# sherholz/mitsuba-path-guiding

Hardware: AMD Instinct MI355X
Metric: Mpaths/sec + equal-spp RMSE vs CPU ref, ajar-door scene at 1/2/4/8 GPUs (higher is better)
Workload: dtype f32; 1 GPU; C3 ajar_door 1280x720, guided SD-tree, 5 training iterations (1..16 spp) + 1024 spp render; scene=ajar_door, triangles=58864, width=1280, height=720, spp=1024, parallelism=tile-shard x1, no exchange (one rank)

## Files before the change

mitsuba-path-guiding_amd/csrc/pg_host.cpp:

```cpp
#include <hip/hip_runtime.h>
#include <rccl/rccl.h>

#include <algorithm>
#include <atomic>
#include <chrono>
#include <cmath>
#include <cstdio>
#include <cstdlib>
#include <cstring>
#include <limits>
#include <string>
#include <vector>

#include "../../include/pg_capi.h"
#include "pg_bvh.h"
#include "pg_envmap.h"
#include "pg_kernels.h"
#include "pg_layout.h"
#include "pg_rtrans.h"
#include "pg_sdtree.h"

namespace {

constexpr uint32_t kStackDepth = 48;
// ... 475 lines not shown
        (void)hipEventCreate(&e.b);
        pool.push_back(e);
    }
    return pool[l->evused[l->evcur]++];
}

bool raySortEnabled() {
    static const bool on = [] {
        const char *e = std::getenv("PG_RAY_SORT");
        return e && std::atoi(e) != 0;
    }();
    return on;
}
constexpr uint32_t kRaySortMinShard = 1024;

uint32_t tailPaths() {
    static const uint32_t n = [] {
        const char *e = std::getenv("PG_TAIL_PATHS");
        return e ? (uint32_t)std::strtoul(e, nullptr, 10) : (uint32_t)1 << 17;
    }();
    return n;
}

int vertexSlots(const Ctx *c, bool rec) { return rec ? std::max(0, std::min(c->cfg.record_max_vertices, 64)) : 0; }

void releasePaths(Ctx *c) {
    for (int li = 0; li < c->nlanes; ++li) {
        Lane &l = c->lanes[li];
        for (DevBuf *b : {&l.ray_o, &l.ray_d, &l.hit, &l.thr, &l.rad, &l.pinfo, &l.sh_d, &l.sh_c,
                          &l.vtx, &l.q0, &l.q1, &l.qs, &l.qp, &l.class_q, &l.aov, &l.qkey, &l.qsorted})
// ... 1302 lines not shown
    uint32_t nextLayer = 0, nextPix = 0, nextChunk = 0;
    uint32_t filmNext = 0;
    HIPC(c, hipEventRecord(c->pass_start, c->stream));
    HIPC(c, hipEventRecord(c->film_order, c->stream));
    c->rec_bound = c->rec_host_count;

    auto lqueue = [](const Lane &l, uint32_t *items, uint32_t *counts) {
        return Queue{items, counts, pg_queue_stride(l.P)};
    };
    auto classQueues = [&](const Lane &l, uint32_t *cb, Queue *cls) {
        for (int k = 0; k < PG_CLASS_ROWS; ++k)
            cls[k] = lqueue(l, k < PG_NUM_CLASSES ? l.class_q.as<uint32_t>() + (size_t)k * PG_QSHARDS * pg_queue_stride(l.P)
                                                 : nullptr,
                            cb + kClassCounts + k * PG_QSHARDS);
    };
    auto launchTrace = [&](Lane &l, const Queue *shq, const Queue *pq) -> pg_status {
        uint32_t *cb = l.counters.as<uint32_t>() + (size_t)kBounceWords * l.b;
        Queue cls[PG_CLASS_ROWS];
        classQueues(l, cb, cls);
        EventPair et{};
        if (evt) et = nextEvents(&l, shq ? KT_RAYS : KT_TRACE);
        if (evt) HIPC(c, hipEventRecord(et.a, l.stream));
        const Queue tq = lqueue(l, l.sorted ? l.qsorted.as<uint32_t>() : (l.b & 1) ? l.q1.as<uint32_t>() : l.q0.as<uint32_t>(),
                                cb);
        if (shq) pg_launch_rays(l.stream, g, sc, pathView(&l), tq, l.bound, cls, *shq, l.bound, *pq);
        else pg_launch_trace(l.stream, g, sc, pathView(&l), tq, l.bound, cls, l.b == 0);
        if (evt) HIPC(c, hipEventRecord(et.b, l.stream));
        HIPC(c, hipMemcpyAsync(l.h_counts + (size_t)kBounceWords * l.b + kClassCounts, cb + kClassCounts,
                               PG_CLASS_ROWS * PG_QSHARDS * 4, hipMemcpyDeviceToHost, l.stream));
        HIPC(c, hipEventRecord(l.ready, l.stream));
        return PG_OK;
    };
    auto collectStats = [&](Lane &l) -> pg_status {
        if (!l.stats_pending) return PG_OK;
        HIPC(c, hipEventSynchronize(l.done));
        for (uint32_t k = 0; k < l.stats_bounces; ++k)
            for (int sh = 0; sh < PG_QSHARDS; ++sh)
            {
                c->stats.shadow_rays += l.h_stats[(size_t)kBounceWords * k + kShadowCounts + sh];
                c->probes += l.h_stats[(size_t)kBounceWords * k + kProbeCounts + sh];
                c->stats.shadow_rays += l.h_stats[(size_t)kBounceWords * k + kDropCounts + sh];
// ... 45 lines not shown
        l.n = np * nl;
        nextPix += np;
        if (nextPix >= npix) {
            nextPix = 0;
            nextLayer += nl;
        }
        l.b = 0;
        l.sorted = false;
        l.bound = pg_camera_bound(pg_camera_banded(bands, l.np), l.np, l.nl);
        l.active = true;
        l.traced = false;
        l.chunk = nextChunk++;
        HIPC(c, hipStreamWaitEvent(l.stream, c->pass_start, 0));
        HIPC(c, hipMemsetAsync(l.counters.p, 0, (size_t)kBounceWords * (maxBounces + 1) * 4, l.stream));
        HIPC(c, hipMemsetAsync(l.tail_stats.p, 0, kTailStats * 8, l.stream));
        pg_launch_camera(l.stream, g, pathView(&l), c->d_band_pixels.as<uint32_t>(), l.pb, l.np, l.nl,
                         sample_offset + l.layer0, lqueue(l, l.q0.as<uint32_t>(), l.counters.as<uint32_t>()), bands);
        return launchTrace(l, nullptr, nullptr);
    };
    auto finishChunk = [&](Lane &l) -> pg_status {
        pg_status st;
        if ((st = collectStats(l))) return st;
        const PathDev pv = pathView(&l);
        HIPC(c, hipMemcpyAsync(l.h_stats, l.counters.p, (size_t)kBounceWords * l.b * 4, hipMemcpyDeviceToHost, l.stream));
        HIPC(c, hipMemcpyAsync(l.h_tail, l.tail_stats.p, kTailStats * 8, hipMemcpyDeviceToHost, l.stream));
        HIPC(c, hipStreamWaitEvent(l.stream, c->film_order, 0));
        pg_launch_film(l.stream, g, sc, pv, c->d_band_pixels.as<uint32_t>(), l.pb, l.np, l.nl, c->film.as<float4>(),
                       c->film_sq.as<float4>(), c->aov_albedo.as<float4>(), c->aov_normal.as<float4>());
        if (c->filtered)
            launchFilmFiltered(c, l.stream, g, sc, pv, c->d_band_pixels.as<uint32_t>(), l.pb, l.np, l.nl,
                               sample_offset + l.layer0);
        if (rec) {
// ... 43 lines not shown
            if (k < PG_NUM_CLASSES) clsMax[k] = m;
        }
        {
            uint64_t t = 0;
            for (int w = 0; w < PG_CLASS_ROWS * PG_QSHARDS; ++w) t += hc[w];
            l.used_cur.push_back(t);
        }
        ++l.b;
        const uint32_t tailMax = c->cfg.tail_paths < 0 ? 0u : c->cfg.tail_paths > 0 ? (uint32_t)c->cfg.tail_paths : tailPaths();
        const bool tail = nlive > 0 && nlive <= tailMax && l.b < maxBounces;
        if (tail) {
            const uint32_t *cbt = l.counters.as<uint32_t>() + (size_t)kBounceWords * (l.b - 1);
            const Queue tq = lqueue(l, l.sorted ? l.qsorted.as<uint32_t>()
                                                : ((l.b - 1) & 1) ? l.q1.as<uint32_t>() : l.q0.as<uint32_t>(),
                                    const_cast<uint32_t *>(cbt));
            pg_launch_tail(l.stream, g, sc, sd, pathView(&l), tq, l.bound, l.tail_stats.as<unsigned long long>());
            c->stats.tail_launches += 1;
        }
        if (nlive == 0 || tail || l.b >= maxBounces) {
            l.traced = true;
            for (bool progress = true; progress;) {
                progress = false;
                for (Lane &o : c->lanes)
                    if (o.active && o.traced && o.chunk == filmNext) {
                        ++filmNext;
                        pg_status st = finishChunk(o);
                        if (st) return st;
                        progress = true;
                    }
            }
            return PG_OK;
// ... 647 lines not shown
```

mitsuba-path-guiding_amd/csrc/pg_kernels.h:

```cpp
#pragma once
#include <hip/hip_runtime.h>
#include <stdint.h>

#include "pg_layout.h"

struct SceneDev {
    const float4 *nodes;
    const float4 *tris;
    const float4 *wnodes;
    const float4 *wtris;
    const float4 *tshade;
    const uint8_t *tclass;
    const GMat *mats;
    const GEmitter *ems;
    const float4 *emtri;
    const float *emcdf;
    const GEnv *env;
    uint32_t top_nodes;
    uint32_t num_em_boxes;
    float em_absmax;
    float em_box[PG_EMBOX_MAX][6];
    uint32_t num_blockers;
    float absmax;
    uint32_t *blk_counts;
// ... 65 lines not shown
struct Queue {
    uint32_t *items;
    uint32_t *counts;
    uint32_t stride;
    uint16_t *keys = nullptr;
    uint32_t *dropped = nullptr;
};
#define PG_RAY_SORT_BINS 4096
__host__ __device__ inline uint32_t pg_queue_stride(uint32_t capacity) {
    return 64u * ((capacity + 4095u) / 4096u + (uint32_t)(((uint64_t)capacity * 7u + (1u << 24) - 1u) >> 24) + 2u);
}
__host__ __device__ inline uint32_t pg_camera_shard_count(uint32_t n, uint32_t s) {
    int rem = (int)(n & 4095u) - 64 * (int)s;
    return 64u * (n >> 12) + (uint32_t)(rem < 0 ? 0 : rem > 64 ? 64 : rem);
}
constexpr uint32_t kBandMinPixels = 4096;
__host__ __device__ inline uint32_t pg_band_start(uint32_t r, uint32_t npix) {
    return (uint32_t)(((uint64_t)r * npix + 7u) / 8u);
}
__host__ __device__ inline uint32_t pg_banded_shard_count(uint32_t npix, uint32_t nlayers, uint32_t s) {
    const uint32_t r = s & 7u, j = s >> 3;
    const uint32_t m = (pg_band_start(r + 1, npix) - pg_band_start(r, npix)) * nlayers;
    const int rem = (int)(m & 511u) - 64 * (int)j;
    return 64u * (m >> 9) + (uint32_t)(rem < 0 ? 0 : rem > 64 ? 64 : rem);
}
__host__ __device__ inline bool pg_camera_banded(bool bands, uint32_t npix) { return bands && npix >= kBandMinPixels; }
__host__ __device__ inline uint32_t pg_camera_count(bool banded, uint32_t npix, uint32_t nlayers, uint32_t s) {
    return banded ? pg_banded_shard_count(npix, nlayers, s) : pg_camera_shard_count(npix * nlayers, s);
}
inline uint32_t pg_camera_bound(bool banded, uint32_t npix, uint32_t nlayers) {
    uint32_t b = 0;
    for (uint32_t s = 0; s < 64; ++s) {
        const uint32_t c = pg_camera_count(banded, npix, nlayers, s);
        b = c > b ? c : b;
    }
    return b;
}

void pg_launch_camera(hipStream_t s, const GParams &g, const PathDev &p, const uint32_t *local_pixels,
                      uint32_t pix_begin, uint32_t npix, uint32_t nlayers, uint32_t sample_base, Queue q, bool banded);
void pg_launch_trace(hipStream_t s, const GParams &g, const SceneDev &sc, const PathDev &p, Queue q, uint32_t max_shard,
                     const Queue *class_queues, bool first_bounce);
void pg_launch_shade_class(hipStream_t s, int cls, const GParams &g, const SceneDev &sc, const SDDev &sd,
                           const PathDev &p, Queue in, uint32_t max_shard, Queue out, Queue shadow, Queue probe);
void pg_launch_shade_all(hipStream_t s, const GParams &g, const SceneDev &sc, const SDDev &sd, const PathDev &p,
                         const Queue *class_queues, const uint32_t *max_shard, Queue out, Queue shq, Queue probe);
void pg_launch_rays(hipStream_t s, const GParams &g, const SceneDev &sc, const PathDev &p, Queue q, uint32_t max_shard,
                    const Queue *class_queues, Queue shq, uint32_t max_shadow_shard, Queue probe);
void pg_launch_shadow(hipStream_t s, const GParams &g, const SceneDev &sc, const PathDev &p, Queue q, uint32_t max_shard);
void pg_launch_probe(hipStream_t s, const SceneDev &sc, const PathDev &p, Queue probe, uint32_t max_shard,
                     const Queue *class_queues);
void pg_launch_tail(hipStream_t s, const GParams &g, const SceneDev &sc, const SDDev &sd, const PathDev &p, Queue q,
                    uint32_t max_shard, unsigned long long *stats);
void pg_launch_ray_sort(hipStream_t s, Queue q, uint32_t max_shard, uint32_t *sorted_items, uint32_t *hist,
                        uint32_t bins = PG_RAY_SORT_BINS);
void pg_launch_film(hipStream_t s, const GParams &g, const SceneDev &sc, const PathDev &p, const uint32_t *local_pixels,
                    uint32_t pix_begin, uint32_t npix, uint32_t nlayers, float4 *film_rgbw, float4 *film_sumsq,
                    float4 *aov_albedo = nullptr, float4 *aov_normal = nullptr);
struct FilmFilter {
    float radius, scale;
    int32_t border;
    uint32_t tile;
    const float *values;
    unsigned long long *acc;
    const uint32_t *tile_first;
    const uint2 *tile_origin;
};
inline size_t pg_film_filter_lds_bytes(uint32_t tile, int32_t border) {
// ... 43 lines not shown
```

mitsuba-path-guiding_amd/csrc/pg_kernels.hip:

```cpp
#include <algorithm>
#include <cstdlib>

#include "pg_trace.h"

#ifndef SHADE_LDS_MATS
#define SHADE_LDS_MATS 0
#endif
#ifndef PG_RAYS_LDS_TOP
#define PG_RAYS_LDS_TOP 0
#endif
#if PG_BVH4
#define PG_TOP_NODE_F4 PG_QNODE_F4
#define PG_TOP_TILE_F4 (PG_BVH4_TOP_NODES * PG_QNODE_F4)
#else
#define PG_TOP_NODE_F4 PG_BVH_NODE_F4
#define PG_TOP_TILE_F4 (PG_BVH_TOP_NODES * PG_BVH_NODE_F4)
#endif
#ifndef PG_TRACE_LDS_TOP
#define PG_TRACE_LDS_TOP 0
#endif

__global__ __launch_bounds__(256) void k_camera(GParams g, PathDev p, const uint32_t *__restrict__ local_pixels,
                                                uint32_t pix_begin, uint32_t npix, uint32_t nlayers,
                                                uint32_t sample_base, Queue q, bool banded) {
    uint32_t slot = blockIdx.x * blockDim.x + threadIdx.x;
    const uint32_t n = npix * nlayers;
    if (slot < PG_QSHARDS) q.counts[slot] = pg_camera_count(banded, npix, nlayers, slot);
    if (slot >= n) return;
    uint32_t layer = slot / npix, lp = slot - layer * npix;
    uint32_t pix = local_pixels[pix_begin + lp];
    uint32_t sample = sample_base + layer;
    uint32_t key = rngKey(pix, g.seed);
    float jx, jy;
    rng2(key, sample, 0, jx, jy);
    float px = (float)(pix % g.width) + jx, py = (float)(pix / g.width) + jy;
    float sx = px / (float)g.width, sy = py / (float)g.height;
    f3 nearP = mk((1.0f - 2.0f * sx) * g.tan_half, (1.0f - 2.0f * sy) / g.aspect * g.tan_half, 1.0f);
    f3 d = normalize(nearP);
    float invZ = 1.0f / d.z;
    f3 left = mk(g.cam_left[0], g.cam_left[1], g.cam_left[2]);
    f3 up = mk(g.cam_up[0], g.cam_up[1], g.cam_up[2]);
    f3 dir = mk(g.cam_dir[0], g.cam_dir[1], g.cam_dir[2]);
    f3 wd = left * d.x + up * d.y + dir * d.z;
    stS(&p.ray_o[slot], make_float4(g.cam_o[0], g.cam_o[1], g.cam_o[2], g.near_clip * invZ));
    stS(&p.ray_d[slot], f4(wd, g.far_clip * invZ));
    stS(&p.rad[slot], make_float4(0.f, 0.f, 0.f, 0.f));
    stS(&p.pinfo[slot], make_uint4(pix, sample, 1u | (PF_EMITTED_QUERY << 16), 0u));
    if (banded) {
        const uint32_t r = (uint32_t)(((uint64_t)lp * 8u) / npix);
        const uint32_t b0 = pg_band_start(r, npix), m = pg_band_start(r + 1, npix) - b0;
        const uint32_t k = layer * m + (lp - b0);
        q.items[(r + 8u * ((k >> 6) & 7u)) * q.stride + (((k >> 9) << 6) | (k & 63u))] = slot;
    } else {
        q.items[((slot >> 6) & 63u) * q.stride + (((slot >> 12) << 6) | (slot & 63u))] = slot;
    }
}

__device__ __forceinline__ f3 bsdfAlbedo(const GMat &M) {
    const f3 diff = mk(M.diff[0], M.diff[1], M.diff[2]), spec = mk(M.spec[0], M.spec[1], M.spec[2]);
    const f3 trans = mk(M.trans[0], M.trans[1], M.trans[2]);
    switch (M.model) {
        case PG_BSDF_DIFFUSE: return diff;
        case PG_BSDF_CONDUCTOR:
        case PG_BSDF_ROUGHCONDUCTOR: return spec;
        case PG_BSDF_DIELECTRIC: return trans * 0.5f + spec * (1 - 0.5f);
        case PG_BSDF_ROUGHDIELECTRIC: return spec * 0.5f + trans * (1 - 0.5f);
        case PG_BSDF_PLASTIC: return diff * 0.5f + spec * (1 - 0.5f);
        case PG_BSDF_ROUGHPLASTIC: return spec * 0.5f + diff * (1 - 0.5f);
        default: return mk1(0.f);
    }
// ... 53 lines not shown
        const int c = __shfl(cls, leader);
        const unsigned long long mine = __ballot(cls == c);
        const Queue &cq = cqs.q[c];
        uint32_t b = 0;
        if (lane == leader) b = atomicAdd(cq.counts + s, (uint32_t)__popcll(mine));
        b = __shfl(b, leader);
        if (cls == c && c < PG_NUM_CLASSES)
            cq.items[(size_t)s * cq.stride + b + __popcll(mine & ((1ull << lane) - 1ull))] = slot;
        pending &= ~mine;
    }
}

#ifndef PG_CLOSEST_WIDE
#define PG_CLOSEST_WIDE 0
#endif
template <bool ENV, bool LTOP, bool CAM, bool WIDE = false>
__device__ __forceinline__ void traceRows(const GParams &g, const SceneDev &sc, const PathDev &p, const Queue &q,
                                          const ClassQueues &cqs, float4 *first, uint32_t bid, uint32_t nblk,
                                          const TStack &stk, const float4 *top, int ntop) {
    const uint32_t s = bid & (PG_QSHARDS - 1);
    const uint32_t n = q.counts[s];
    const uint32_t *items = q.items + (size_t)s * q.stride;
    for (uint32_t base = (bid / PG_QSHARDS) * TRACE_BLOCK; base < n; base += nblk / PG_QSHARDS * TRACE_BLOCK) {
        const uint32_t i = base + threadIdx.x;
        int cls = -1;
        uint32_t slot = 0;
        if (i < n) {
            slot = items[i];
            float4 o = ldS(&p.ray_o[slot]), d = ldS(&p.ray_d[slot]);
            slot |= rayDoomed(o) ? 0x80000000u : 0u;
            const float tmin = fabsf(o.w);
            float tmax = CAM ? d.w : __builtin_huge_valf();
            uint32_t tri = 0xFFFFFFFFu;
            float u = 0, v = 0;
            bool h;
            if constexpr (WIDE)
                h = traverseWide<false>(sc.wnodes, sc.wtris, xyz(o), xyz(d), tmin, tmax, tri, u, v,
                                        WStack{stk.lds, stk.ovf, stk.ostride});
            else
                h = traverse<false, LTOP>(sc.nodes, sc.tris, xyz(o), xyz(d), tmin, tmax, tri, u, v, stk, top, ntop);
            const bool doomed = (slot >> 31) != 0;
            slot &= 0x7FFFFFFFu;
            float4 hr = make_float4(h ? tmax : 0.0f, __uint_as_float(h ? tri : 0xFFFFFFFFu), u, v);
            if (first) first[slot] = hr;
            if (ENV && !h) {
                const f3 e = envEscapeRadiance(g, sc, p, slot, xyz(d), CAM ? kCameraWord : p.pinfo[slot].z, d.w);
                hr = make_float4(e.x, hr.y, e.y, e.z);
            }
            cls = hitClass(sc, h, tri, doomed, hr);
            stS(&p.hit[slot], hr);
        }
        classAppend(cls, slot, cqs, s);
    }
}

#ifndef PG_TRACE_PERSIST
#define PG_TRACE_PERSIST 0
#endif
#ifndef PG_TRACE_REFILL
#define PG_TRACE_REFILL 24
#endif
// ... 93 lines not shown
            slotB = items[ib];
            const float4 o = ldS(&p.ray_o[slotB]), d = ldS(&p.ray_d[slotB]);
            doomedB = rayDoomed(o);
            woPdfB = d.w;
            walk4Start(b, xyz(o), xyz(d), fabsf(o.w), __builtin_huge_valf());
        }
        walk4Pair(a, b, sc.nodes, sc.tris, sa, sb);
        int ca = -1, cb = -1;
        if (ia < n) finishWalk<ENV>(g, sc, p, a, slotA, doomedA, woPdfA, first, ca);
        if (ib < n) finishWalk<ENV>(g, sc, p, b, slotB, doomedB, woPdfB, first, cb);
        classAppend(ca, slotA, cqs, s);
        classAppend(cb, slotB, cqs, s);
    }
}

template <bool ENV, bool CAM>
__global__ __launch_bounds__(TRACE_BLOCK) void k_trace(GParams g, SceneDev sc, PathDev p, Queue q, ClassQueues cqs,
                                                       float4 *first) {
    __shared__ uint32_t stack[LDS_STACK * TRACE_BLOCK];
    __shared__ float4 top[(PG_TRACE_LDS_TOP ? PG_TOP_TILE_F4 : 1)];
    const int ntop = PG_TRACE_LDS_TOP ? (int)sc.top_nodes : 0;
    if (PG_TRACE_LDS_TOP) {
        for (uint32_t k = threadIdx.x; k < (uint32_t)ntop * PG_TOP_NODE_F4; k += TRACE_BLOCK) top[k] = sc.nodes[k];
        __syncthreads();
    }
    traceRows<ENV, PG_TRACE_LDS_TOP != 0, CAM>(g, sc, p, q, cqs, first, blockIdx.x, gridDim.x, threadStack(stack, p.stack_ovf),
                                          top, ntop);
}

__device__ __forceinline__ float shadowTmin(float4 o) {
    return kEpsilon * fmaxf(fmaxf(fabsf(o.x), fabsf(o.y)), fabsf(o.z));
}

template <class T>
__device__ __forceinline__ void waveKeyedAdd(T *base, uint32_t key, T v, bool valid);
__device__ __forceinline__ bool blockerRowCounted(uint32_t row) { return row % PG_BLOCKER_SAMPLE == 0; }
__device__ __forceinline__ void shadowAdd(const PathDev &p, uint32_t slot) {
    float4 c = ldS(&p.sh_c[slot]);
    float4 L = ldS(&p.rad[slot]);
    stS(&p.rad[slot], make_float4(L.x + c.x, L.y + c.y, L.z + c.z, L.w));
    uint32_t vi = __float_as_uint(c.w);
    if (vi != 0xFFFFFFFFu) {
// ... 89 lines not shown
        shadowRows<COUNT>(sc, p, shq, blockIdx.x - trace_blocks, shadow_blocks, threadWideStack(stack, p.stack_ovf));
    } else {
        __shared__ float4 top[PG_RAYS_LDS_TOP ? PG_TOP_TILE_F4 : 1];
        const int ntop = PG_RAYS_LDS_TOP ? (int)sc.top_nodes : 0;
        if (PG_RAYS_LDS_TOP) {
            for (uint32_t k = threadIdx.x; k < (uint32_t)ntop * PG_TOP_NODE_F4; k += TRACE_BLOCK) top[k] = sc.nodes[k];
            __syncthreads();
        }
        const TStack sa = threadStack(stack, p.stack_ovf);
        if (PG_TRACE_PAIR && !PG_RAYS_LDS_TOP && !PG_CLOSEST_WIDE && PG_BVH4 && PG_QNODE_QUANT)
            traceRowsPair<ENV>(g, sc, p, q, cqs, nullptr, blockIdx.x, trace_blocks, sa,
                               TStack{sa.lds + LDS_STACK * TRACE_BLOCK, sa.ovf + (size_t)kPairRing * sa.ostride, sa.ostride});
        else if (PG_TRACE_PERSIST && !PG_RAYS_LDS_TOP && !PG_CLOSEST_WIDE && PG_BVH4 && PG_QNODE_QUANT)
            traceRowsPersist<ENV>(g, sc, p, q, cqs, nullptr, blockIdx.x, trace_blocks, sa);
        else
            traceRows<ENV, PG_RAYS_LDS_TOP != 0, false, PG_CLOSEST_WIDE != 0>(g, sc, p, q, cqs, nullptr, blockIdx.x, trace_blocks,
                                                 sa, top, ntop);
    }
#else
    if (blockIdx.x < shadow_blocks)
        shadowRows<COUNT>(sc, p, shq, blockIdx.x, shadow_blocks, threadWideStack(stack, p.stack_ovf));
    else
        traceRows<ENV, false, false>(g, sc, p, q, cqs, nullptr, blockIdx.x - shadow_blocks,
                              gridDim.x - probe_blocks - shadow_blocks, threadStack(stack, p.stack_ovf), nullptr, 0);
#endif
}

__device__ __forceinline__ uint32_t rayOrderKey(const SDDev &sd, f3 o, f3 d) {
    const float inv = 8.0f / sd.extent;
    const int cx = min(max((int)((o.x - sd.lo[0]) * inv), 0), 7);
    const int cy = min(max((int)((o.y - sd.lo[1]) * inv), 0), 7);
    const int cz = min(max((int)((o.z - sd.lo[2]) * inv), 0), 7);
    uint32_t m = 0;
    for (int b = 0; b < 3; ++b)
        m |= (((cx >> b) & 1) << (3 * b)) | (((cy >> b) & 1) << (3 * b + 1)) | (((cz >> b) & 1) << (3 * b + 2));
    const uint32_t oct = (d.x < 0 ? 1u : 0u) | (d.y < 0 ? 2u : 0u) | (d.z < 0 ? 4u : 0u);
    return (oct << 9) | m;
}
// ... 75 lines not shown
            if (!haveL) {
                L = xyz(ldS(&p.rad[slot]));
                haveL = true;
            }
        };
        if (PG_WATCH) loadL();
        float eta = T4.w;
        uint32_t tri = __float_as_uint(hv.y);
        if (tri == 0xFFFFFFFFu) break;
        const uint32_t key = rngKey(pix, g.seed);
        f3 rd = xyz(rd4);
#if PG_SD_PREFETCH
        uint32_t jCell = 0xFFFFFFFFu, jSpec = 0;
        uint4 metaSpec = make_uint4(0, 0, 0, 0);
        if (CAN_GUIDE && g.guiding && sd.built) {
            const float4 ro = ldS(&p.ray_o[slot]);
            const SDView sv0 = sdv(sd);
            jCell = sdJumpCell(sv0, mk(ro.x + hv.x * rd.x, ro.y + hv.x * rd.y, ro.z + hv.x * rd.z));
            jSpec = sd.jump[jCell];
        }
#endif
        Hit h;
        fetchHit(sc, tri, hv.z, hv.w, rd, h);
#if PG_SD_PREFETCH
        if (CAN_GUIDE && g.guiding && sd.built) metaSpec = sd.meta[(jSpec & 0x80000000u) ? (jSpec & 0x7FFFFFFFu) : 0u];
#endif
        WSET(0, depth);
        WSET(1, __float_as_uint(sc.tshade[(size_t)PG_TRI_SHADE_STRIDE * tri + 2].w));
        WSET3(2, h.p);
        f3 Le = mk1(0.f);
        if (h.emitter >= 0 && dot(h.shN, -rd) > 0) {
// ... 385 lines not shown
        case PG_CLASS_ROUGHDIELECTRIC:
            shadeOne<PG_BSDF_ROUGHDIELECTRIC, true, ENV>(g, sc, sd, p, slot, sc.mats, false, alive, shadow, probe, rk, blocked);
            break;
        case PG_CLASS_PLASTIC: shadeOne<PG_BSDF_PLASTIC, false, ENV>(g, sc, sd, p, slot, sc.mats, false, alive, shadow, probe, rk, blocked); break;
        case PG_CLASS_ROUGHPLASTIC:
            shadeOne<PG_BSDF_ROUGHPLASTIC, true, ENV>(g, sc, sd, p, slot, sc.mats, false, alive, shadow, probe, rk, blocked);
            break;
        default: shadeOne<-1, false, ENV>(g, sc, sd, p, slot, sc.mats, false, alive, shadow, probe, rk, blocked);
    }
}
#ifndef PG_TAIL_WAVES
#define PG_TAIL_WAVES 0
#endif
template <bool ENV, bool COUNT = false>
__global__ __launch_bounds__(TRACE_BLOCK) __attribute__((amdgpu_waves_per_eu(PG_TAIL_WAVES > 0 ? PG_TAIL_WAVES : 1))) void k_tail(GParams g, SceneDev sc, SDDev sd, PathDev p, Queue q,
                                                      unsigned long long *stats) {
    __shared__ uint32_t stack[2 * WIDE_LDS_STACK * TRACE_BLOCK];
    const TStack stk = threadStack(stack, p.stack_ovf);
    const WStack wstk = threadWideStack(stack, p.stack_ovf);
    const uint32_t s = blockIdx.x & (PG_QSHARDS - 1);
    const uint32_t rows = gridDim.x / PG_QSHARDS;
    const uint32_t n = q.counts[s];
    uint32_t segs = 0, esc = 0, shadows = 0, culled = 0, probes = 0, drops = 0;
    for (uint32_t i = (blockIdx.x / PG_QSHARDS) * TRACE_BLOCK + threadIdx.x; i < n; i += rows * TRACE_BLOCK) {
        const uint32_t slot = q.items[(size_t)s * q.stride + i];
        uint32_t tri = __float_as_uint(ldS(&p.hit[slot]).y);
        while (tri != 0xFFFFFFFFu) {
            bool alive = false, shadow = false, probe = false;
            uint32_t blocked = 0;
            tailShade<ENV>(g, sc, sd, p, slot, tri, alive, shadow, probe, blocked);
            if (!ENV && blocked) {
                ++shadows;
                ++drops;
                if (COUNT && blockerRowCounted(i / TRACE_BLOCK)) {
                    atomicAdd(sc.blk_counts + (blocked - 1u), 1u);
                    atomicAdd(sc.blk_total, 1u);
                }
            }
            if (shadow) {
                ++shadows;
// ... 541 lines not shown
}
uint64_t pg_trace_rays_threads(uint64_t n) { return (uint64_t)blocks(n, TRACE_BLOCK) * TRACE_BLOCK; }

void pg_launch_camera(hipStream_t s, const GParams &g, const PathDev &p, const uint32_t *local_pixels,
                      uint32_t pix_begin, uint32_t npix, uint32_t nlayers, uint32_t sample_base, Queue q, bool banded) {
    uint64_t n = (uint64_t)npix * nlayers;
    if (!n) return;
    hipLaunchKernelGGL(k_camera, dim3(blocks(n, 256)), dim3(256), 0, s, g, p, local_pixels, pix_begin, npix, nlayers,
                       sample_base, q, pg_camera_banded(banded, npix));
}
static inline dim3 shardGrid(uint32_t max_shard, uint32_t block, uint32_t max_rows) {
    const uint32_t rows = blocks(max_shard, block);
    return dim3(PG_QSHARDS * (rows < max_rows ? rows : max_rows));
}
void pg_launch_trace(hipStream_t s, const GParams &g, const SceneDev &sc, const PathDev &p, Queue q, uint32_t max_shard,
                     const Queue *class_queues, bool first_bounce) {
    if (!max_shard) return;
    ClassQueues cq;
    for (int c = 0; c < PG_CLASS_ROWS; ++c) cq.q[c] = class_queues[c];
    const dim3 grid = shardGrid(max_shard, TRACE_BLOCK, TRACE_MAX_BLOCKS / PG_QSHARDS);
    float4 *first = first_bounce ? p.aov : nullptr;
    if (first_bounce) {
        if (sc.env) hipLaunchKernelGGL((k_trace<true, true>), grid, dim3(TRACE_BLOCK), 0, s, g, sc, p, q, cq, first);
        else hipLaunchKernelGGL((k_trace<false, true>), grid, dim3(TRACE_BLOCK), 0, s, g, sc, p, q, cq, first);
    } else {
        if (sc.env) hipLaunchKernelGGL((k_trace<true, false>), grid, dim3(TRACE_BLOCK), 0, s, g, sc, p, q, cq, first);
        else hipLaunchKernelGGL((k_trace<false, false>), grid, dim3(TRACE_BLOCK), 0, s, g, sc, p, q, cq, first);
    }
}
template <bool ENV>
static void launchShade(hipStream_t s, int cls, dim3 grid, const GParams &g, const SceneDev &sc, const SDDev &sd,
                        const PathDev &p, Queue in, Queue out, Queue shq, Queue pq) {
    const dim3 block(SHADE_BLOCK);
    switch (cls) {
        case PG_CLASS_DIFFUSE:
            hipLaunchKernelGGL((k_shade<PG_BSDF_DIFFUSE, true, ENV>), grid, block, 0, s, g, sc, sd, p, in, out, shq, pq);
            break;
        case PG_CLASS_ROUGHCONDUCTOR:
            hipLaunchKernelGGL((k_shade<PG_BSDF_ROUGHCONDUCTOR, true, ENV>), grid, block, 0, s, g, sc, sd, p, in, out, shq, pq);
            break;
        case PG_CLASS_ROUGHDIELECTRIC:
            hipLaunchKernelGGL((k_shade<PG_BSDF_ROUGHDIELECTRIC, true, ENV>), grid, block, 0, s, g, sc, sd, p, in, out, shq, pq);
// ... 53 lines not shown
void pg_launch_probe(hipStream_t s, const SceneDev &sc, const PathDev &p, Queue pq, uint32_t max_shard,
                     const Queue *class_queues) {
    if (!max_shard) return;
    ClassQueues cq;
    for (int c = 0; c < PG_CLASS_ROWS; ++c) cq.q[c] = class_queues[c];
    hipLaunchKernelGGL(k_probe, shardGrid(max_shard, TRACE_BLOCK, TRACE_MAX_BLOCKS / PG_QSHARDS), dim3(TRACE_BLOCK), 0, s,
                       sc, p, pq, cq);
}
void pg_launch_shadow(hipStream_t s, const GParams &g, const SceneDev &sc, const PathDev &p, Queue q, uint32_t max_shard) {
    if (!max_shard) return;
    const dim3 grid = shardGrid(max_shard, TRACE_BLOCK, TRACE_MAX_BLOCKS / PG_QSHARDS);
    if (blockersCounted(g, sc)) hipLaunchKernelGGL(k_shadow<true>, grid, dim3(TRACE_BLOCK), 0, s, sc, p, q);
    else hipLaunchKernelGGL(k_shadow<false>, grid, dim3(TRACE_BLOCK), 0, s, sc, p, q);
}
void pg_launch_tail(hipStream_t s, const GParams &g, const SceneDev &sc, const SDDev &sd, const PathDev &p, Queue q,
                    uint32_t max_shard, unsigned long long *stats) {
    if (!max_shard) return;
    const dim3 grid = shardGrid(max_shard, TRACE_BLOCK, TRACE_MAX_BLOCKS / PG_QSHARDS);
    if (sc.env) hipLaunchKernelGGL(k_tail<true>, grid, dim3(TRACE_BLOCK), 0, s, g, sc, sd, p, q, stats);
    else if (blockersCounted(g, sc)) hipLaunchKernelGGL((k_tail<false, true>), grid, dim3(TRACE_BLOCK), 0, s, g, sc, sd, p, q, stats);
    else hipLaunchKernelGGL(k_tail<false>, grid, dim3(TRACE_BLOCK), 0, s, g, sc, sd, p, q, stats);
}
template <uint32_t BINS>
static void raySort(hipStream_t s, Queue q, uint32_t max_shard, uint32_t *sorted_items, uint32_t *hist) {
    (void)hipMemsetAsync(hist, 0, (size_t)PG_QSHARDS * BINS * 4, s);
    const dim3 grid(PG_QSHARDS * blocks(max_shard, RSORT_TILE));
    hipLaunchKernelGGL(k_rsort_hist<BINS>, grid, dim3(256), 0, s, q, hist);
    hipLaunchKernelGGL(k_rsort_scan<BINS>, dim3(PG_QSHARDS), dim3(256), 0, s, hist);
    hipLaunchKernelGGL(k_rsort_scatter<BINS>, grid, dim3(256), 0, s, q, hist, sorted_items);
}
void pg_launch_ray_sort(hipStream_t s, Queue q, uint32_t max_shard, uint32_t *sorted_items, uint32_t *hist,
                        uint32_t bins) {
    if (!max_shard) return;
    if (bins == 512) raySort<512>(s, q, max_shard, sorted_items, hist);
    else raySort<PG_RAY_SORT_BINS>(s, q, max_shard, sorted_items, hist);
}
// ... 111 lines not shown
```

Baseline: 847.2 Mpaths/s.

## Fuse camera ray generation into first-bounce trace kernel and drop ray_o store

```diff
diff --git a/mitsuba-path-guiding_amd/csrc/pg_host.cpp b/mitsuba-path-guiding_amd/csrc/pg_host.cpp
--- a/mitsuba-path-guiding_amd/csrc/pg_host.cpp
+++ b/mitsuba-path-guiding_amd/csrc/pg_host.cpp
@@ -513,6 +513,11 @@
 }
 constexpr uint32_t kRaySortMinShard = 1024;
 
+bool cameraFusion() {
+    static const bool on = !std::getenv("PG_NO_CAMERA_FUSION");
+    return on;
+}
+
 uint32_t tailPaths() {
     static const uint32_t n = [] {
         const char *e = std::getenv("PG_TAIL_PATHS");
@@ -1845,6 +1850,10 @@
                                                  : nullptr,
                             cb + kClassCounts + k * PG_QSHARDS);
     };
+    auto cameraChunk = [&](const Lane &l) {
+        return CameraChunk{c->d_band_pixels.as<uint32_t>(), l.pb, l.np, l.nl, sample_offset + l.layer0,
+                           pg_camera_banded(bands, l.np)};
+    };
     auto launchTrace = [&](Lane &l, const Queue *shq, const Queue *pq) -> pg_status {
         uint32_t *cb = l.counters.as<uint32_t>() + (size_t)kBounceWords * l.b;
         Queue cls[PG_CLASS_ROWS];
@@ -1855,7 +1864,10 @@
         const Queue tq = lqueue(l, l.sorted ? l.qsorted.as<uint32_t>() : (l.b & 1) ? l.q1.as<uint32_t>() : l.q0.as<uint32_t>(),
                                 cb);
         if (shq) pg_launch_rays(l.stream, g, sc, pathView(&l), tq, l.bound, cls, *shq, l.bound, *pq);
-        else pg_launch_trace(l.stream, g, sc, pathView(&l), tq, l.bound, cls, l.b == 0);
+        else if (l.b == 0 && cameraFusion()) {
+            const CameraChunk cam = cameraChunk(l);
+            pg_launch_trace(l.stream, g, sc, pathView(&l), tq, l.bound, cls, true, &cam);
+        } else pg_launch_trace(l.stream, g, sc, pathView(&l), tq, l.bound, cls, l.b == 0);
         if (evt) HIPC(c, hipEventRecord(et.b, l.stream));
         HIPC(c, hipMemcpyAsync(l.h_counts + (size_t)kBounceWords * l.b + kClassCounts, cb + kClassCounts,
                                PG_CLASS_ROWS * PG_QSHARDS * 4, hipMemcpyDeviceToHost, l.stream));
@@ -1931,8 +1943,9 @@
         HIPC(c, hipStreamWaitEvent(l.stream, c->pass_start, 0));
         HIPC(c, hipMemsetAsync(l.counters.p, 0, (size_t)kBounceWords * (maxBounces + 1) * 4, l.stream));
         HIPC(c, hipMemsetAsync(l.tail_stats.p, 0, kTailStats * 8, l.stream));
-        pg_launch_camera(l.stream, g, pathView(&l), c->d_band_pixels.as<uint32_t>(), l.pb, l.np, l.nl,
-                         sample_offset + l.layer0, lqueue(l, l.q0.as<uint32_t>(), l.counters.as<uint32_t>()), bands);
+        if (!cameraFusion())
+            pg_launch_camera(l.stream, g, pathView(&l), c->d_band_pixels.as<uint32_t>(), l.pb, l.np, l.nl,
+                             sample_offset + l.layer0, lqueue(l, l.q0.as<uint32_t>(), l.counters.as<uint32_t>()), bands);
         return launchTrace(l, nullptr, nullptr);
     };
     auto finishChunk = [&](Lane &l) -> pg_status {
@@ -2006,7 +2019,10 @@
             const Queue tq = lqueue(l, l.sorted ? l.qsorted.as<uint32_t>()
                                                 : ((l.b - 1) & 1) ? l.q1.as<uint32_t>() : l.q0.as<uint32_t>(),
                                     const_cast<uint32_t *>(cbt));
-            pg_launch_tail(l.stream, g, sc, sd, pathView(&l), tq, l.bound, l.tail_stats.as<unsigned long long>());
+            const bool camRows = l.b == 1 && cameraFusion();
+            const CameraChunk cam = cameraChunk(l);
+            pg_launch_tail(l.stream, g, sc, sd, pathView(&l), tq, l.bound, l.tail_stats.as<unsigned long long>(),
+                           camRows ? &cam : nullptr);
             c->stats.tail_launches += 1;
         }
         if (nlive == 0 || tail || l.b >= maxBounces) {
diff --git a/mitsuba-path-guiding_amd/csrc/pg_kernels.h b/mitsuba-path-guiding_amd/csrc/pg_kernels.h
--- a/mitsuba-path-guiding_amd/csrc/pg_kernels.h
+++ b/mitsuba-path-guiding_amd/csrc/pg_kernels.h
@@ -103,6 +103,13 @@
     int rem = (int)(n & 4095u) - 64 * (int)s;
     return 64u * (n >> 12) + (uint32_t)(rem < 0 ? 0 : rem > 64 ? 64 : rem);
 }
+__host__ __device__ inline void pg_camera_place(uint32_t slot, uint32_t &s, uint32_t &i) {
+    s = (slot >> 6) & 63u;
+    i = ((slot >> 12) << 6) | (slot & 63u);
+}
+__host__ __device__ inline uint32_t pg_camera_slot(uint32_t s, uint32_t i) {
+    return ((i >> 6) << 12) | (s << 6) | (i & 63u);
+}
 constexpr uint32_t kBandMinPixels = 4096;
 __host__ __device__ inline uint32_t pg_band_start(uint32_t r, uint32_t npix) {
     return (uint32_t)(((uint64_t)r * npix + 7u) / 8u);
@@ -112,6 +119,20 @@
     const uint32_t m = (pg_band_start(r + 1, npix) - pg_band_start(r, npix)) * nlayers;
     const int rem = (int)(m & 511u) - 64 * (int)j;
     return 64u * (m >> 9) + (uint32_t)(rem < 0 ? 0 : rem > 64 ? 64 : rem);
+}
+__host__ __device__ inline void pg_banded_place(uint32_t npix, uint32_t layer, uint32_t lp, uint32_t &s, uint32_t &i) {
+    const uint32_t r = (uint32_t)(((uint64_t)lp * 8u) / npix);
+    const uint32_t b0 = pg_band_start(r, npix), m = pg_band_start(r + 1, npix) - b0;
+    const uint32_t k = layer * m + (lp - b0);
+    s = r + 8u * ((k >> 6) & 7u);
+    i = ((k >> 9) << 6) | (k & 63u);
+}
+__host__ __device__ inline void pg_banded_item(uint32_t npix, uint32_t s, uint32_t i, uint32_t &layer, uint32_t &lp) {
+    const uint32_t r = s & 7u, j = s >> 3;
+    const uint32_t b0 = pg_band_start(r, npix), m = pg_band_start(r + 1, npix) - b0;
+    const uint32_t k = ((i >> 6) << 9) | (j << 6) | (i & 63u);
+    layer = k / m;
+    lp = b0 + (k - layer * m);
 }
 __host__ __device__ inline bool pg_camera_banded(bool bands, uint32_t npix) { return bands && npix >= kBandMinPixels; }
 __host__ __device__ inline uint32_t pg_camera_count(bool banded, uint32_t npix, uint32_t nlayers, uint32_t s) {
@@ -128,8 +149,13 @@
 
 void pg_launch_camera(hipStream_t s, const GParams &g, const PathDev &p, const uint32_t *local_pixels,
                       uint32_t pix_begin, uint32_t npix, uint32_t nlayers, uint32_t sample_base, Queue q, bool banded);
+struct CameraChunk {
+    const uint32_t *local_pixels;
+    uint32_t pix_begin, npix, nlayers, sample_base;
+    bool banded;
+};
 void pg_launch_trace(hipStream_t s, const GParams &g, const SceneDev &sc, const PathDev &p, Queue q, uint32_t max_shard,
-                     const Queue *class_queues, bool first_bounce);
+                     const Queue *class_queues, bool first_bounce, const CameraChunk *gen = nullptr);
 void pg_launch_shade_class(hipStream_t s, int cls, const GParams &g, const SceneDev &sc, const SDDev &sd,
                            const PathDev &p, Queue in, uint32_t max_shard, Queue out, Queue shadow, Queue probe);
 void pg_launch_shade_all(hipStream_t s, const GParams &g, const SceneDev &sc, const SDDev &sd, const PathDev &p,
@@ -140,7 +166,7 @@
 void pg_launch_probe(hipStream_t s, const SceneDev &sc, const PathDev &p, Queue probe, uint32_t max_shard,
                      const Queue *class_queues);
 void pg_launch_tail(hipStream_t s, const GParams &g, const SceneDev &sc, const SDDev &sd, const PathDev &p, Queue q,
-                    uint32_t max_shard, unsigned long long *stats);
+                    uint32_t max_shard, unsigned long long *stats, const CameraChunk *gen = nullptr);
 void pg_launch_ray_sort(hipStream_t s, Queue q, uint32_t max_shard, uint32_t *sorted_items, uint32_t *hist,
                         uint32_t bins = PG_RAY_SORT_BINS);
 void pg_launch_film(hipStream_t s, const GParams &g, const SceneDev &sc, const PathDev &p, const uint32_t *local_pixels,
diff --git a/mitsuba-path-guiding_amd/csrc/pg_kernels.hip b/mitsuba-path-guiding_amd/csrc/pg_kernels.hip
--- a/mitsuba-path-guiding_amd/csrc/pg_kernels.hip
+++ b/mitsuba-path-guiding_amd/csrc/pg_kernels.hip
@@ -20,6 +20,37 @@
 #define PG_TRACE_LDS_TOP 0
 #endif
 
+__device__ __forceinline__ void cameraRay(const GParams &g, uint32_t pix, uint32_t sample, f3 &wd, float &invZ) {
+    uint32_t key = rngKey(pix, g.seed);
+    float jx, jy;
+    rng2(key, sample, 0, jx, jy);
+    float px = (float)(pix % g.width) + jx, py = (float)(pix / g.width) + jy;
+    float sx = px / (float)g.width, sy = py / (float)g.height;
+    f3 nearP = mk((1.0f - 2.0f * sx) * g.tan_half, (1.0f - 2.0f * sy) / g.aspect * g.tan_half, 1.0f);
+    f3 d = normalize(nearP);
+    invZ = 1.0f / d.z;
+    f3 left = mk(g.cam_left[0], g.cam_left[1], g.cam_left[2]);
+    f3 up = mk(g.cam_up[0], g.cam_up[1], g.cam_up[2]);
+    f3 dir = mk(g.cam_dir[0], g.cam_dir[1], g.cam_dir[2]);
+    wd = left * d.x + up * d.y + dir * d.z;
+}
+__device__ __forceinline__ uint32_t cameraRowSlot(const CameraChunk &cam, uint32_t s, uint32_t i, uint32_t &layer,
+                                                  uint32_t &lp) {
+    if (cam.banded) {
+        pg_banded_item(cam.npix, s, i, layer, lp);
+        return layer * cam.npix + lp;
+    }
+    const uint32_t slot = pg_camera_slot(s, i);
+    layer = slot / cam.npix;
+    lp = slot - layer * cam.npix;
+    return slot;
+}
+__device__ __forceinline__ void storeCameraRows(const PathDev &p, uint32_t slot, uint32_t pix, uint32_t sample,
+                                                float4 d) {
+    stS(&p.ray_d[slot], d);
+    stS(&p.rad[slot], make_float4(0.f, 0.f, 0.f, 0.f));
+    stS(&p.pinfo[slot], make_uint4(pix, sample, 1u | (PF_EMITTED_QUERY << 16), 0u));
+}
 __global__ __launch_bounds__(256) void k_camera(GParams g, PathDev p, const uint32_t *__restrict__ local_pixels,
                                                 uint32_t pix_begin, uint32_t npix, uint32_t nlayers,
                                                 uint32_t sample_base, Queue q, bool banded) {
@@ -30,30 +61,15 @@
     uint32_t layer = slot / npix, lp = slot - layer * npix;
     uint32_t pix = local_pixels[pix_begin + lp];
     uint32_t sample = sample_base + layer;
-    uint32_t key = rngKey(pix, g.seed);
-    float jx, jy;
-    rng2(key, sample, 0, jx, jy);
-    float px = (float)(pix % g.width) + jx, py = (float)(pix / g.width) + jy;
-    float sx = px / (float)g.width, sy = py / (float)g.height;
-    f3 nearP = mk((1.0f - 2.0f * sx) * g.tan_half, (1.0f - 2.0f * sy) / g.aspect * g.tan_half, 1.0f);
-    f3 d = normalize(nearP);
-    float invZ = 1.0f / d.z;
-    f3 left = mk(g.cam_left[0], g.cam_left[1], g.cam_left[2]);
-    f3 up = mk(g.cam_up[0], g.cam_up[1], g.cam_up[2]);
-    f3 dir = mk(g.cam_dir[0], g.cam_dir[1], g.cam_dir[2]);
-    f3 wd = left * d.x + up * d.y + dir * d.z;
+    f3 wd;
+    float invZ;
+    cameraRay(g, pix, sample, wd, invZ);
     stS(&p.ray_o[slot], make_float4(g.cam_o[0], g.cam_o[1], g.cam_o[2], g.near_clip * invZ));
-    stS(&p.ray_d[slot], f4(wd, g.far_clip * invZ));
-    stS(&p.rad[slot], make_float4(0.f, 0.f, 0.f, 0.f));
-    stS(&p.pinfo[slot], make_uint4(pix, sample, 1u | (PF_EMITTED_QUERY << 16), 0u));
-    if (banded) {
-        const uint32_t r = (uint32_t)(((uint64_t)lp * 8u) / npix);
-        const uint32_t b0 = pg_band_start(r, npix), m = pg_band_start(r + 1, npix) - b0;
-        const uint32_t k = layer * m + (lp - b0);
-        q.items[(r + 8u * ((k >> 6) & 7u)) * q.stride + (((k >> 9) << 6) | (k & 63u))] = slot;
-    } else {
-        q.items[((slot >> 6) & 63u) * q.stride + (((slot >> 12) << 6) | (slot & 63u))] = slot;
-    }
+    storeCameraRows(p, slot, pix, sample, f4(wd, g.far_clip * invZ));
+    uint32_t s, i;
+    if (banded) pg_banded_place(npix, layer, lp, s, i);
+    else pg_camera_place(slot, s, i);
+    q.items[s * q.stride + i] = slot;
 }
 
 __device__ __forceinline__ f3 bsdfAlbedo(const GMat &M) {
@@ -137,23 +153,44 @@
 #ifndef PG_CLOSEST_WIDE
 #define PG_CLOSEST_WIDE 0
 #endif
-template <bool ENV, bool LTOP, bool CAM, bool WIDE = false>
+constexpr int kRowsBounce = 0;
+constexpr int kRowsCamera = 1;
+constexpr int kRowsCameraGen = 2;
+template <bool ENV, bool LTOP, int CAM, bool WIDE = false>
 __device__ __forceinline__ void traceRows(const GParams &g, const SceneDev &sc, const PathDev &p, const Queue &q,
                                           const ClassQueues &cqs, float4 *first, uint32_t bid, uint32_t nblk,
-                                          const TStack &stk, const float4 *top, int ntop) {
+                                          const TStack &stk, const float4 *top, int ntop,
+                                          const CameraChunk &cam = CameraChunk{}) {
     const uint32_t s = bid & (PG_QSHARDS - 1);
-    const uint32_t n = q.counts[s];
+    const uint32_t n = CAM == kRowsCameraGen ? pg_camera_count(cam.banded, cam.npix, cam.nlayers, s) : q.counts[s];
     const uint32_t *items = q.items + (size_t)s * q.stride;
     for (uint32_t base = (bid / PG_QSHARDS) * TRACE_BLOCK; base < n; base += nblk / PG_QSHARDS * TRACE_BLOCK) {
         const uint32_t i = base + threadIdx.x;
         int cls = -1;
         uint32_t slot = 0;
         if (i < n) {
-            slot = items[i];
-            float4 o = ldS(&p.ray_o[slot]), d = ldS(&p.ray_d[slot]);
+            float4 o, d;
+            if constexpr (CAM == kRowsCameraGen) {
+                GParams gc = g;
+                CameraChunk cc = cam;
+                asm volatile("" : "+s"(gc.width), "+s"(gc.height), "+s"(gc.aspect), "+s"(cc.npix));
+                uint32_t layer, lp;
+                slot = cameraRowSlot(cc, s, i, layer, lp);
+                const uint32_t pix = cc.local_pixels[cc.pix_begin + lp], sample = cc.sample_base + layer;
+                f3 wd;
+                float invZ;
+                cameraRay(gc, pix, sample, wd, invZ);
+                o = make_float4(g.cam_o[0], g.cam_o[1], g.cam_o[2], g.near_clip * invZ);
+                d = f4(wd, g.far_clip * invZ);
+                storeCameraRows(p, slot, pix, sample, d);
+            } else {
+                slot = items[i];
+                o = ldS(&p.ray_o[slot]);
+                d = ldS(&p.ray_d[slot]);
+            }
             slot |= rayDoomed(o) ? 0x80000000u : 0u;
             const float tmin = fabsf(o.w);
-            float tmax = CAM ? d.w : __builtin_huge_valf();
+            float tmax = CAM != kRowsBounce ? d.w : __builtin_huge_valf();
             uint32_t tri = 0xFFFFFFFFu;
             float u = 0, v = 0;
             bool h;
@@ -167,7 +204,7 @@
             float4 hr = make_float4(h ? tmax : 0.0f, __uint_as_float(h ? tri : 0xFFFFFFFFu), u, v);
             if (first) first[slot] = hr;
             if (ENV && !h) {
-                const f3 e = envEscapeRadiance(g, sc, p, slot, xyz(d), CAM ? kCameraWord : p.pinfo[slot].z, d.w);
+                const f3 e = envEscapeRadiance(g, sc, p, slot, xyz(d), CAM != kRowsBounce ? kCameraWord : p.pinfo[slot].z, d.w);
                 hr = make_float4(e.x, hr.y, e.y, e.z);
             }
             cls = hitClass(sc, h, tri, doomed, hr);
@@ -291,9 +328,9 @@
     }
 }
 
-template <bool ENV, bool CAM>
-__global__ __launch_bounds__(TRACE_BLOCK) void k_trace(GParams g, SceneDev sc, PathDev p, Queue q, ClassQueues cqs,
-                                                       float4 *first) {
+template <bool ENV, int CAM>
+__global__ __launch_bounds__(TRACE_BLOCK) __attribute__((amdgpu_waves_per_eu(!ENV && CAM == kRowsCameraGen ? 6 : 1))) void k_trace(GParams g, SceneDev sc, PathDev p, Queue q, ClassQueues cqs,
+                                                       float4 *first, CameraChunk cam) {
     __shared__ uint32_t stack[LDS_STACK * TRACE_BLOCK];
     __shared__ float4 top[(PG_TRACE_LDS_TOP ? PG_TOP_TILE_F4 : 1)];
     const int ntop = PG_TRACE_LDS_TOP ? (int)sc.top_nodes : 0;
@@ -302,7 +339,7 @@
         __syncthreads();
     }
     traceRows<ENV, PG_TRACE_LDS_TOP != 0, CAM>(g, sc, p, q, cqs, first, blockIdx.x, gridDim.x, threadStack(stack, p.stack_ovf),
-                                          top, ntop);
+                                          top, ntop, cam);
 }
 
 __device__ __forceinline__ float shadowTmin(float4 o) {
@@ -422,14 +459,14 @@
         else if (PG_TRACE_PERSIST && !PG_RAYS_LDS_TOP && !PG_CLOSEST_WIDE && PG_BVH4 && PG_QNODE_QUANT)
             traceRowsPersist<ENV>(g, sc, p, q, cqs, nullptr, blockIdx.x, trace_blocks, sa);
         else
-            traceRows<ENV, PG_RAYS_LDS_TOP != 0, false, PG_CLOSEST_WIDE != 0>(g, sc, p, q, cqs, nullptr, blockIdx.x, trace_blocks,
+            traceRows<ENV, PG_RAYS_LDS_TOP != 0, kRowsBounce, PG_CLOSEST_WIDE != 0>(g, sc, p, q, cqs, nullptr, blockIdx.x, trace_blocks,
                                                  sa, top, ntop);
     }
 #else
     if (blockIdx.x < shadow_blocks)
         shadowRows<COUNT>(sc, p, shq, blockIdx.x, shadow_blocks, threadWideStack(stack, p.stack_ovf));
     else
-        traceRows<ENV, false, false>(g, sc, p, q, cqs, nullptr, blockIdx.x - shadow_blocks,
+        traceRows<ENV, false, kRowsBounce>(g, sc, p, q, cqs, nullptr, blockIdx.x - shadow_blocks,
                               gridDim.x - probe_blocks - shadow_blocks, threadStack(stack, p.stack_ovf), nullptr, 0);
 #endif
 }
@@ -535,7 +572,7 @@
         uint32_t jCell = 0xFFFFFFFFu, jSpec = 0;
         uint4 metaSpec = make_uint4(0, 0, 0, 0);
         if (CAN_GUIDE && g.guiding && sd.built) {
-            const float4 ro = ldS(&p.ray_o[slot]);
+            const float4 ro = depth == 1 ? make_float4(g.cam_o[0], g.cam_o[1], g.cam_o[2], 0.0f) : ldS(&p.ray_o[slot]);
             const SDView sv0 = sdv(sd);
             jCell = sdJumpCell(sv0, mk(ro.x + hv.x * rd.x, ro.y + hv.x * rd.y, ro.z + hv.x * rd.z));
             jSpec = sd.jump[jCell];
@@ -951,16 +988,17 @@
 #endif
 template <bool ENV, bool COUNT = false>
 __global__ __launch_bounds__(TRACE_BLOCK) __attribute__((amdgpu_waves_per_eu(PG_TAIL_WAVES > 0 ? PG_TAIL_WAVES : 1))) void k_tail(GParams g, SceneDev sc, SDDev sd, PathDev p, Queue q,
-                                                      unsigned long long *stats) {
+                                                      unsigned long long *stats, CameraChunk cam) {
     __shared__ uint32_t stack[2 * WIDE_LDS_STACK * TRACE_BLOCK];
     const TStack stk = threadStack(stack, p.stack_ovf);
     const WStack wstk = threadWideStack(stack, p.stack_ovf);
     const uint32_t s = blockIdx.x & (PG_QSHARDS - 1);
     const uint32_t rows = gridDim.x / PG_QSHARDS;
-    const uint32_t n = q.counts[s];
+    const uint32_t n = cam.npix ? pg_camera_count(cam.banded, cam.npix, cam.nlayers, s) : q.counts[s];
     uint32_t segs = 0, esc = 0, shadows = 0, culled = 0, probes = 0, drops = 0;
     for (uint32_t i = (blockIdx.x / PG_QSHARDS) * TRACE_BLOCK + threadIdx.x; i < n; i += rows * TRACE_BLOCK) {
-        const uint32_t slot = q.items[(size_t)s * q.stride + i];
+        uint32_t layer, lp;
+        const uint32_t slot = cam.npix ? cameraRowSlot(cam, s, i, layer, lp) : q.items[(size_t)s * q.stride + i];
         uint32_t tri = __float_as_uint(ldS(&p.hit[slot]).y);
         while (tri != 0xFFFFFFFFu) {
             bool alive = false, shadow = false, probe = false;
@@ -1532,18 +1570,22 @@
     return dim3(PG_QSHARDS * (rows < max_rows ? rows : max_rows));
 }
 void pg_launch_trace(hipStream_t s, const GParams &g, const SceneDev &sc, const PathDev &p, Queue q, uint32_t max_shard,
-                     const Queue *class_queues, bool first_bounce) {
+                     const Queue *class_queues, bool first_bounce, const CameraChunk *gen) {
     if (!max_shard) return;
     ClassQueues cq;
     for (int c = 0; c < PG_CLASS_ROWS; ++c) cq.q[c] = class_queues[c];
     const dim3 grid = shardGrid(max_shard, TRACE_BLOCK, TRACE_MAX_BLOCKS / PG_QSHARDS);
     float4 *first = first_bounce ? p.aov : nullptr;
-    if (first_bounce) {
-        if (sc.env) hipLaunchKernelGGL((k_trace<true, true>), grid, dim3(TRACE_BLOCK), 0, s, g, sc, p, q, cq, first);
-        else hipLaunchKernelGGL((k_trace<false, true>), grid, dim3(TRACE_BLOCK), 0, s, g, sc, p, q, cq, first);
+    const CameraChunk cam = gen ? *gen : CameraChunk{};
+    if (first_bounce && gen) {
+        if (sc.env) hipLaunchKernelGGL((k_trace<true, kRowsCameraGen>), grid, dim3(TRACE_BLOCK), 0, s, g, sc, p, q, cq, first, cam);
+        else hipLaunchKernelGGL((k_trace<false, kRowsCameraGen>), grid, dim3(TRACE_BLOCK), 0, s, g, sc, p, q, cq, first, cam);
+    } else if (first_bounce) {
+        if (sc.env) hipLaunchKernelGGL((k_trace<true, kRowsCamera>), grid, dim3(TRACE_BLOCK), 0, s, g, sc, p, q, cq, first, cam);
+        else hipLaunchKernelGGL((k_trace<false, kRowsCamera>), grid, dim3(TRACE_BLOCK), 0, s, g, sc, p, q, cq, first, cam);
     } else {
-        if (sc.env) hipLaunchKernelGGL((k_trace<true, false>), grid, dim3(TRACE_BLOCK), 0, s, g, sc, p, q, cq, first);
-        else hipLaunchKernelGGL((k_trace<false, false>), grid, dim3(TRACE_BLOCK), 0, s, g, sc, p, q, cq, first);
+        if (sc.env) hipLaunchKernelGGL((k_trace<true, kRowsBounce>), grid, dim3(TRACE_BLOCK), 0, s, g, sc, p, q, cq, first, cam);
+        else hipLaunchKernelGGL((k_trace<false, kRowsBounce>), grid, dim3(TRACE_BLOCK), 0, s, g, sc, p, q, cq, first, cam);
     }
 }
 template <bool ENV>
@@ -1627,12 +1669,13 @@
     else hipLaunchKernelGGL(k_shadow<false>, grid, dim3(TRACE_BLOCK), 0, s, sc, p, q);
 }
 void pg_launch_tail(hipStream_t s, const GParams &g, const SceneDev &sc, const SDDev &sd, const PathDev &p, Queue q,
-                    uint32_t max_shard, unsigned long long *stats) {
+                    uint32_t max_shard, unsigned long long *stats, const CameraChunk *gen) {
     if (!max_shard) return;
     const dim3 grid = shardGrid(max_shard, TRACE_BLOCK, TRACE_MAX_BLOCKS / PG_QSHARDS);
-    if (sc.env) hipLaunchKernelGGL(k_tail<true>, grid, dim3(TRACE_BLOCK), 0, s, g, sc, sd, p, q, stats);
-    else if (blockersCounted(g, sc)) hipLaunchKernelGGL((k_tail<false, true>), grid, dim3(TRACE_BLOCK), 0, s, g, sc, sd, p, q, stats);
-    else hipLaunchKernelGGL(k_tail<false>, grid, dim3(TRACE_BLOCK), 0, s, g, sc, sd, p, q, stats);
+    const CameraChunk cam = gen ? *gen : CameraChunk{};
+    if (sc.env) hipLaunchKernelGGL(k_tail<true>, grid, dim3(TRACE_BLOCK), 0, s, g, sc, sd, p, q, stats, cam);
+    else if (blockersCounted(g, sc)) hipLaunchKernelGGL((k_tail<false, true>), grid, dim3(TRACE_BLOCK), 0, s, g, sc, sd, p, q, stats, cam);
+    else hipLaunchKernelGGL(k_tail<false>, grid, dim3(TRACE_BLOCK), 0, s, g, sc, sd, p, q, stats, cam);
 }
 template <uint32_t BINS>
 static void raySort(hipStream_t s, Queue q, uint32_t max_shard, uint32_t *sorted_items, uint32_t *hist) {
```

Measured after the change: 855.3 Mpaths/s, median of 6. No clear change (+1.0%).
